# spcl/arrow-matrix

Measured on NVIDIA H100. Metric: iterated SpMM GFLOP/s (k=128), higher is better.
Workload: dtype f32

## Files before the change

arrow_matrix_b200/_lib.py:

```python
from __future__ import annotations

import ctypes
import os
from ctypes import (POINTER, byref, c_char_p, c_double, c_float, c_int, c_int32, c_int64, c_size_t, c_void_p)
from typing import Optional, Sequence, Tuple

import numpy as np

_HERE = os.path.dirname(os.path.abspath(__file__))
LIB_PATH = os.path.join(_HERE, "libarrow_b200.so")

ACCUMULATE = 1
F32, F64 = 0, 1
I32 = 2
B1 = 3
BITS = "bits"
_DTYPE_CODE = {np.dtype(np.float32): F32, np.dtype(np.float64): F64}
_TILE_CODE = {**_DTYPE_CODE, np.dtype(np.int32): I32}
_CODE_TILE = {**{c: dt for dt, c in _TILE_CODE.items()}, B1: BITS}
VARIANT_AUTO, VARIANT_DIRECT, VARIANT_SHFL, VARIANT_TMA, VARIANT_TILES = -1, 0, 1, 2, 3
SR_PLUS_TIMES, SR_MIN_PLUS, SR_MAX_PLUS, SR_OR_AND = 0, 1, 2, 3
SEMIRINGS = {"plus_times": SR_PLUS_TIMES, "min_plus": SR_MIN_PLUS, "max_plus": SR_MAX_PLUS, "or_and": SR_OR_AND}
IPC_HANDLE_BYTES = 80

# ... 8 lines not shown
    "arrow_event_record", "arrow_event_wait",
    "arrow_spmm", "arrow_spmm_add", "arrow_gather_rows", "arrow_gather_rows_multi",
    "arrow_ipc_export", "arrow_ipc_import", "arrow_peer_barrier",
    "arrow_timer_start", "arrow_timer_stop", "arrow_timer_elapsed_ms", "arrow_launch_count", "arrow_l2_flush",
    "arrow_ptrtable_upload", "arrow_ptrtable_free", "arrow_spmm_ex", "arrow_push_rows", "arrow_reduce_rows",
    "arrow_graph_begin", "arrow_graph_end", "arrow_graph_launch", "arrow_graph_free",
    "arrow_host_alloc_numa", "arrow_bind_thread_to_device_numa", "arrow_preload_kernels",
    "arrow_csr_upload_f64", "arrow_dense_alloc_dtype", "arrow_dense_dtype",
    "arrow_spmm_sr", "arrow_gather_rows_sr", "arrow_dense_count_diff",
    "arrow_spmm_sr_witness", "arrow_tile_rows", "arrow_tile_rows_rule", "arrow_bits_mark_new",
    "arrow_adj_build", "arrow_adj_free", "arrow_adj_info", "arrow_adj_d2h", "arrow_bits_mark_frontier",
    "arrow_bits_push_frontier", "arrow_adj_build_weighted", "arrow_adj_values_d2h", "arrow_sr_mark_frontier",
    "arrow_sr_push_frontier", "arrow_adj_build_in", "arrow_bits_parents", "arrow_bits_path_counts",
    "arrow_adj_keep_record", "arrow_bits_dependencies", "arrow_bits_fill_f64", "arrow_dense_row_sum",
    "arrow_adj_build_loopfree", "arrow_wpaths_counts", "arrow_wpaths_dependencies",
]
ABI_VERSION = 12


class ArrowError(RuntimeError):
    def __init__(self, code: int, message: str):
        super().__init__(f"libarrow_b200 error {code}: {message}")
        self.code = code


_lib = None


def load_library(build_if_missing: bool = True) -> ctypes.CDLL:
    global _lib
    if _lib is not None:
        return _lib
# ... 12 lines not shown
    I, I64 = c_int, c_int64
    pI, pI64 = POINTER(c_int), POINTER(c_int64)
    sig = {
        "arrow_b200_abi_version": (c_int, []),
        "arrow_ctx_create": (c_int, [I, P, POINTER(P)]),
        "arrow_ctx_destroy": (None, [P]),
        "arrow_last_error": (c_char_p, [P]),
        "arrow_sync": (c_int, [P]),
        "arrow_device_info": (c_int, [P, pI, pI64, pI64]),
        "arrow_set_tuning": (c_int, [P, I, I]),
        "arrow_set_option": (c_int, [P, I, I]),
        "arrow_csr_upload": (c_int, [P, I64, I64, I64, P, I, P, I, P, pI]),
        "arrow_csr_free": (c_int, [P, I]),
        "arrow_csr_info": (c_int, [P, I, pI64, pI64, pI64, pI64, pI64]),
        "arrow_csr_remap_columns": (c_int, [P, I, I, I64, pI]),
        "arrow_map_upload": (c_int, [P, P, I64, I64, pI]),
        "arrow_map_free": (c_int, [P, I]),
        "arrow_map_compose": (c_int, [P, I, I, pI]),
        "arrow_map_invert": (c_int, [P, I, I64, pI]),
        "arrow_map_d2h": (c_int, [P, I, P, I64]),
        "arrow_dense_alloc": (c_int, [P, I64, I, pI]),
        "arrow_dense_free": (c_int, [P, I]),
        "arrow_dense_fill": (c_int, [P, I, c_float]),
        "arrow_dense_h2d": (c_int, [P, I, I64, I64, P]),
        "arrow_dense_d2h": (c_int, [P, I, I64, I64, P]),
        "arrow_dense_copy": (c_int, [P, I, I64, I, I64, I64]),
        "arrow_dense_ptr": (c_int, [P, I, POINTER(P), pI64, pI]),
        "arrow_dense_wrap": (c_int, [P, P, I64, I, pI]),
        "arrow_dense_h2d_lane": (c_int, [P, I, I, I64, I64, P]),
        "arrow_dense_d2h_lane": (c_int, [P, I, I, I64, I64, P]),
        "arrow_lane_wait": (c_int, [P, I, I]),
        "arrow_lane_sync": (c_int, [P, I]),
        "arrow_set_lane": (c_int, [P, I]),
        "arrow_event_record": (c_int, [P, I, I]),
        "arrow_event_wait": (c_int, [P, I, I]),
        "arrow_host_alloc": (c_int, [c_size_t, POINTER(P)]),
        "arrow_host_free": (c_int, [P]),
        "arrow_spmm": (c_int, [P, I, I, I, I, I, I]),
        "arrow_spmm_add": (c_int, [P, I, I, I, I, I, I]),
        "arrow_gather_rows": (c_int, [P, I, I, I, I]),
        "arrow_gather_rows_multi": (c_int, [P, I, pI, pI64, I, I, I]),
        "arrow_ipc_export": (c_int, [P, I, P]),
        "arrow_ipc_import": (c_int, [P, P, I64, I, pI]),
        "arrow_peer_barrier": (c_int, [P, pI, I, I]),
        "arrow_timer_start": (c_int, [P, I]),
        "arrow_timer_stop": (c_int, [P, I]),
        "arrow_timer_elapsed_ms": (c_int, [P, I, POINTER(c_float)]),
        "arrow_launch_count": (c_int, [P, pI64]),
        "arrow_l2_flush": (c_int, [P]),
        "arrow_ptrtable_upload": (c_int, [P, pI, I, P, P, I64, pI]),
        "arrow_ptrtable_free": (c_int, [P, I]),
        "arrow_spmm_ex": (c_int, [P, I, I, I, I64, I, I, I, I, I]),
        "arrow_push_rows": (c_int, [P, pI, pI64, I, I, I]),
        "arrow_reduce_rows": (c_int, [P, I, I, pI, I, I64]),
# ... 226 lines not shown
    def ipc_import(self, handle: bytes, rows: int, k: int) -> "Dense":
        assert len(handle) == IPC_HANDLE_BYTES
        buf = ctypes.create_string_buffer(handle, IPC_HANDLE_BYTES)
        h = c_int()
        self._check(self.lib.arrow_ipc_import(self._h, buf, int(rows), int(k), byref(h)))
        return Dense(self, h.value, int(rows), int(k), owned=False)

    def spmm(self, A: "Csr", X: "Dense", C: "Dense", rowmap: Optional["RowMap"] = None,
             accumulate: bool = False, variant: int = VARIANT_AUTO):
        self._check(self.lib.arrow_spmm(self._h, A.h, X.h, C.h, rowmap.h if rowmap is not None else -1,
                                        ACCUMULATE if accumulate else 0, int(variant)))

    def spmm_add(self, A: "Csr", X: "Dense", C: "Dense", add: "Dense", add_map: "RowMap", variant: int = VARIANT_AUTO):
        self._check(self.lib.arrow_spmm_add(self._h, A.h, X.h, C.h, add.h, add_map.h, int(variant)))

    def spmm_sr(self, A: "Csr", X: "Dense", C: "Dense", add: Optional["Dense"] = None,
                add_map: Optional["RowMap"] = None, semiring: int = SR_PLUS_TIMES):
        self._check(self.lib.arrow_spmm_sr(self._h, A.h, X.h, C.h, add.h if add is not None else -1,
                                           add_map.h if add_map is not None else -1, int(semiring)))

    def spmm_sr_witness(self, A: "Csr", X: "Dense", labels: "Dense", values: Optional["Dense"] = None,
                        add_values: Optional["Dense"] = None, add_labels: Optional["Dense"] = None,
                        add_map: Optional["RowMap"] = None, dist: Optional["Dense"] = None,
                        row_labels: Optional["RowMap"] = None, semiring: int = SR_MIN_PLUS):
        h = lambda o: o.h if o is not None else -1
        self._check(self.lib.arrow_spmm_sr_witness(self._h, A.h, X.h, h(row_labels), h(values), labels.h, h(add_values),
                                                   h(add_labels), h(add_map), h(dist), int(semiring)))

    def spmm_ex(self, A: "Csr", X: "Dense", C: Optional["Dense"] = None, X2: Optional["Dense"] = None, x_split: int = 0,
                out_table: Optional["PtrTable"] = None, add: Optional["Dense"] = None, add_map: Optional["RowMap"] = None,
# ... 216 lines not shown
        self.n_rows, self.n_cols, self.nnz = n_rows, n_cols, nnz
        self.dtype = np.dtype(dtype)

    def info(self):
        v = [c_int64() for _ in range(5)]
        self.ctx._check(self.ctx.lib.arrow_csr_info(self.ctx._h, self.h, *[byref(x) for x in v]))
        return dict(zip(("n_rows", "n_cols", "nnz", "max_row_nnz", "n_long_rows"), (x.value for x in v)))

    def remap_columns(self, m: "RowMap", new_n_cols: int) -> "Csr":
        h = c_int()
        self.ctx._check(self.ctx.lib.arrow_csr_remap_columns(self.ctx._h, self.h, m.h, int(new_n_cols), byref(h)))
        out = Csr(self.ctx, h.value, self.n_rows, int(new_n_cols), self.nnz, self.dtype)
        out._parent = self
        return out

    def free(self):
        self._free("arrow_csr_free")


class RowMap(_Handle):
    def __init__(self, ctx, h, n, limit):
        super().__init__(ctx, h)
        self.n, self.limit = n, limit

    def compose(self, outer: "RowMap") -> "RowMap":
        h = c_int()
        self.ctx._check(self.ctx.lib.arrow_map_compose(self.ctx._h, self.h, outer.h, byref(h)))
        return RowMap(self.ctx, h.value, self.n, outer.limit)

    def invert(self, n_out: int) -> "RowMap":
# ... 95 lines not shown
```

arrow_matrix_b200/csrc/arrow_b200.cu:

```cuda
#include "../../include/arrow_b200.h"

#include <cuda_runtime.h>
#include <ctype.h>
#include <dlfcn.h>
#include <sched.h>
#include <sys/mman.h>
#include <sys/syscall.h>
#include <unistd.h>
#include <stdint.h>
#include <stdarg.h>
#include <stdio.h>
#include <string.h>

#include <cub/device/device_radix_sort.cuh>

#include <algorithm>
#include <map>
#include <mutex>
#include <type_traits>
#include <string>
#include <vector>

namespace {

struct DenseBuf {
    float *p = nullptr;
    int64_t rows = 0;
    int k = 0;
    int dtype = ARROW_F32;
// ... 1609 lines not shown
    bool bad = false;
    for (long long i = (long long)blockIdx.x * blockDim.x + threadIdx.x; i < n; i += stride) {
        const int c = idx[i];
        const int m = (c < 0 || c >= map_n) ? -1 : map[c];
        out[i] = m;
        bad = bad || m < 0;
    }
    if (bad && any_invalid != nullptr) atomicExch(any_invalid, 1);
}

__global__ void k_map_invert(const int *__restrict__ map, long long n, int *__restrict__ out, long long n_out) {
    const long long stride = (long long)gridDim.x * blockDim.x;
    for (long long i = (long long)blockIdx.x * blockDim.x + threadIdx.x; i < n; i += stride) {
        const int q = map[i];
        if (q >= 0 && q < n_out) out[q] = (int)i;
    }
}

struct PeerFlags {
    unsigned int *p[MAX_SRC];
};
__global__ void k_peer_barrier(PeerFlags flags, int rank, int world, unsigned int *epoch_ctr, int *status, long long timeout_clocks) {
    __shared__ unsigned int s_epoch;
    __threadfence_system();
    if (threadIdx.x == 0) {
        s_epoch = *epoch_ctr + 1u;
        *epoch_ctr = s_epoch;
    }
    __syncthreads();
    const unsigned int epoch = s_epoch;
// ... 2486 lines not shown
        if (e == cudaSuccess) e = cudaMemcpyAsync(&h_invalid, flag.p, sizeof(int), cudaMemcpyDeviceToHost, ctx->stream);
        if (e == cudaSuccess) e = cudaStreamSynchronize(ctx->stream);
    }
    if (e != cudaSuccess) {
        cudaFree(d.indices);
        return fail(ctx, ARROW_ERR_CUDA, "column remap failed: %s", cudaGetErrorString(e));
    }
    d.may_skip = c->may_skip || h_invalid != 0;
    const int h = new_slot(ctx->csrs);
    ctx->csrs[h] = d;
    ctx->csrs[csr].children++;
    *csr_out = h;
    return ARROW_OK;
}

int arrow_map_upload(arrow_ctx *ctx, const int64_t *map, int64_t n, int64_t limit, int *map_out) {
    CHECK_CTX(ctx);
    if (!map_out || (n > 0 && !map)) return fail(ctx, ARROW_ERR_ARG, "null pointer argument");
    if (n < 0 || limit < 0 || limit > 2147483647LL || n > 2147483647LL)
        return fail(ctx, ARROW_ERR_RANGE, "map size/limit exceed the int32 device layout");
    IdxMap m;
    m.n = n;
    m.limit = limit;
    CUDA_TRY(ctx, cudaMalloc(&m.p, (size_t)std::max<int64_t>(n, 1) * sizeof(int)));
    cudaError_t e = cudaSuccess;
    if (n > 0) {
        DevTmp wide;
        e = cudaMalloc(&wide.p, (size_t)n * 8);
        if (e == cudaSuccess) e = cudaMemcpyAsync(wide.p, map, (size_t)n * 8, cudaMemcpyHostToDevice, ctx->stream);
        if (e == cudaSuccess) {
// ... 242 lines not shown
    if (len) {
        const bool ok = cudaHostUnregister(ptr) == cudaSuccess;
        munmap(ptr, len);
        return ok ? ARROW_OK : ARROW_ERR_CUDA;
    }
    return cudaFreeHost(ptr) == cudaSuccess ? ARROW_OK : ARROW_ERR_CUDA;
}

struct SpmmCall {
    int csr = -1, x_buf = -1, c_buf = -1;
    int rowmap = -1, flags = 0, variant = ARROW_VARIANT_AUTO;
    int add_buf = -1, add_map = -1;
    int x2_buf = -1;
    int64_t x_split = 0;
    int out_table = -1;
};
static int spmm_impl(arrow_ctx *ctx, const SpmmCall &q);

#define CHECK_POISON(ctx)                                                                                     \
    do {                                                                                                      \
        if ((ctx)->poisoned) return fail((ctx), ARROW_ERR_CUDA, "context is poisoned by a peer-barrier time-out"); \
    } while (0)

int arrow_spmm(arrow_ctx *ctx, int csr, int x_buf, int c_buf, int rowmap, int flags, int variant) {
    SpmmCall q;
    q.csr = csr; q.x_buf = x_buf; q.c_buf = c_buf; q.rowmap = rowmap; q.flags = flags; q.variant = variant;
    return spmm_impl(ctx, q);
}

int arrow_spmm_add(arrow_ctx *ctx, int csr, int x_buf, int c_buf, int add_buf, int add_map, int variant) {
    SpmmCall q;
    q.csr = csr; q.x_buf = x_buf; q.c_buf = c_buf; q.variant = variant; q.add_buf = add_buf; q.add_map = add_map;
    return spmm_impl(ctx, q);
}

int arrow_spmm_ex(arrow_ctx *ctx, int csr, int x_buf, int x2_buf, int64_t x_split, int c_buf, int out_table,
                  int add_buf, int add_map, int variant) {
    SpmmCall q;
    q.csr = csr; q.x_buf = x_buf; q.x2_buf = x2_buf; q.x_split = x_split; q.c_buf = c_buf; q.out_table = out_table;
    q.add_buf = add_buf; q.add_map = add_map; q.variant = variant;
    return spmm_impl(ctx, q);
}

static int spmm_impl(arrow_ctx *ctx, const SpmmCall &q) {
    CHECK_CTX(ctx);
    CHECK_POISON(ctx);
    Csr *A = get_csr(ctx, q.csr);
// ... 75 lines not shown
        a.add_map = am->p;
    }
    if (A->dtype == ARROW_F64) {
        if (X2 || OT) return fail(ctx, ARROW_ERR_UNSUPPORTED, "float64 has no two-part X operand or pointer-table epilogue (one GPU only)");
        if (q.variant != ARROW_VARIANT_AUTO && q.variant != ARROW_VARIANT_TILES)
            return fail(ctx, ARROW_ERR_UNSUPPORTED, "float64 has no kernel variant override (variant %d)", q.variant);
        return spmm_f64(ctx, A, a, rm != nullptr, acc);
    }
    int variant = q.variant;
    if (variant == ARROW_VARIANT_AUTO) variant = pick_variant(k);
    const int vpl_req = (variant >> 4) & 0xF;
    const int rpg_req = (variant >> 8) & 0x3;
    variant &= 0xF;
    if ((a.add_map != nullptr || X2 || OT) && variant != 3) variant = 3;
    if (variant < 0 || variant > 3) return fail(ctx, ARROW_ERR_ARG, "unknown variant %d", variant);
    const bool fused_launch = rm != nullptr || acc || OT != nullptr || X2 != nullptr || a.add_map != nullptr;

    const bool vec_ok = (k % 4 == 0) && k <= 256;
    if (!vec_ok) {
        launch_generic<PlusTimes<float>>(ctx, a, rm != nullptr, acc);
    } else if (variant == 3) {
        if (A->n_tiles[TILE_LIST_SMALL] > 0) {
            TileArgs t;
            t.a = a;
            t.skip = (A->may_skip || ctx->force_skip_path) ? 1 : 0;
            t.ticket = ctx->tile_ticket + 2 * lane;
            t.l2_hints = (rm != nullptr || acc) ? ctx->l2_hints_fused : ctx->l2_hints_plain;
            t.prefetch = fused_launch ? ctx->prefetch_fused : ctx->prefetch_plain;
            TileLaunch L;
            L.out_mode = OT ? OUT_ROWPTR : (rm ? OUT_ROWMAP : OUT_IDENTITY);
            L.acc = acc;
            L.dualx = X2 != nullptr;
            L.vpl_req = vpl_req;
            L.rpg_req = rpg_req;
            int rc = launch_tiles(ctx, t, A, L);
            if (rc != ARROW_OK) return rc;
        }
    } else if (variant == ARROW_VARIANT_TMA && k >= 32 && k <= 128) {
        if (a.k4 <= 32) launch_tma<1>(ctx, a, rm != nullptr, acc);
        else launch_tma<2>(ctx, a, rm != nullptr, acc);
    } else {
        if (variant == ARROW_VARIANT_TMA) variant = ARROW_VARIANT_SHFL;
// ... 1747 lines not shown
```

arrow_matrix_b200/decomp.py:

```python
from __future__ import annotations

from typing import List, Optional, Sequence, Tuple, Union

import numpy as np
from scipy import sparse

Triplet = Tuple[Optional[np.ndarray], np.ndarray, np.ndarray]
Level = Union[sparse.csr_matrix, Triplet]


def level_triplet(level: Level) -> Triplet:
    if isinstance(level, tuple):
        return level
    m = sparse.csr_matrix(level)
    return (m.data, m.indices, m.indptr)


def number_of_blocks(level: Level, width: int) -> int:
    indptr = np.asarray(level_triplet(level)[2])
    nnz_total = int(indptr[-1] - indptr[0])
    if nnz_total == 0:
        raise ValueError("level has no non-zero row")
    last = int(np.searchsorted(indptr, indptr[-1], side="left")) - 1
    return -(-(last + 1) // width)
# ... 96 lines not shown
    assert ip.size == rows + 1
    out_ptr = ip + np.arange(rows + 1, dtype=np.int64)
    nnz = int(out_ptr[-1])
    diag = out_ptr[:-1]
    rest = np.ones(nnz, dtype=bool)
    rest[diag] = False
    idx = np.empty(nnz, dtype=np.result_type(np.asarray(indices).dtype, np.int32))
    idx[diag] = np.arange(rows)
    idx[rest] = indices
    dat = np.empty(nnz, dtype=dtype)
    dat[diag] = value
    dat[rest] = 1 if data is None else data
    return out_ptr, idx, dat


def block_partition(n_blocks: int, parts: int) -> np.ndarray:
    g = np.arange(parts + 1, dtype=np.int64)
    return (g * n_blocks + parts - 1) // parts


def locality_partition(to_prev: np.ndarray, n_blocks: int, width: int, prev_bounds_rows: np.ndarray, parts: int,
                       min_local: float = 0.5, max_skew: float = 4.0) -> Optional[np.ndarray]:
    rows = n_blocks * width
    if n_blocks < 1 or parts < 2:
        return None
    tp = np.asarray(to_prev[:rows])
    valid = tp < int(prev_bounds_rows[-1])
    owner = np.searchsorted(prev_bounds_rows, np.where(valid, tp, 0), side="right") - 1
    blk = np.arange(rows, dtype=np.int64) // width
    votes = np.zeros((n_blocks, parts), dtype=np.int64)
# ... 19 lines not shown
```

arrow_matrix_b200/engine.py:

```python
from __future__ import annotations

from typing import List, Optional, Sequence, Tuple

import numpy as np

from . import _lib
from . import decomp


_PLUS_ZERO = {_lib.SR_PLUS_TIMES: 0.0, _lib.SR_MIN_PLUS: float("inf"), _lib.SR_MAX_PLUS: float("-inf"), _lib.SR_OR_AND: 0.0}
_TIMES_ONE = {_lib.SR_PLUS_TIMES: 1.0, _lib.SR_MIN_PLUS: 0.0, _lib.SR_MAX_PLUS: 0.0, _lib.SR_OR_AND: 1.0}


BFS_PUSH_ALPHA = 8


def bfs_direction(frontier_edges: int, total_nnz: int, alpha: float = BFS_PUSH_ALPHA) -> str:
    return "push" if frontier_edges * alpha < total_nnz else "pull"


SR_PUSH_ALPHA = 9


def semiring_code(semiring: str, dtype, fused_style: str = "gather") -> int:
    if semiring not in _lib.SEMIRINGS:
        raise ValueError(f"unknown semiring {semiring!r}: expected one of {', '.join(_lib.SEMIRINGS)}")
    code = _lib.SEMIRINGS[semiring]
    if code != _lib.SR_PLUS_TIMES:
        if np.dtype(dtype) != np.float32:
            raise ValueError(f"the {semiring} semiring computes in float32, the decomposition is {np.dtype(dtype)}")
        if fused_style != "gather":
            raise ValueError(f"the {semiring} semiring runs the gather style of the fused step, not {fused_style!r}")
    return code


_SCAN_CHUNK = 1 << 24
# ... 2 lines not shown
def _nonpositive_edge(ip, idx, dat, cmap) -> bool:
    ip, idx, dat = np.asarray(ip), np.asarray(idx), np.asarray(dat)
    for e0 in range(0, dat.size, _SCAN_CHUNK):
        e = np.flatnonzero(~(dat[e0:e0 + _SCAN_CHUNK] > 0)) + e0
        if e.size == 0:
            continue
        r, c = np.searchsorted(ip, e, side="right") - 1, idx[e].astype(np.int64)
        ok = (r != c) & (c >= 0)
        if np.any(ok & (cmap[r] >= 0) & (cmap[np.where(ok, c, 0)] >= 0)):
            return True
    return False


class _LevelState:
    __slots__ = ("rows", "n_blocks", "csr", "csr_fused", "to_prev", "to_next_dev", "to_prev_dev", "cmap_dev",
                 "bufs", "xi", "ci", "nnz", "dropped", "cbuf")

    def __init__(self):
        self.csr = self.csr_fused = None
        self.to_prev = None
        self.to_prev_dev = self.to_next_dev = self.cmap_dev = None
        self.bufs = [None, None]
        self.xi = self.ci = 0
        self.cbuf = None


class ArrowEngine:

    def __init__(self, decomposition: Sequence[Tuple[decomp.Level, np.ndarray]], width: int, k: int,
                 block_diagonal: bool = True, device: int = 0, mode: str = "auto", stream: Optional[int] = None,
                 variant: int = _lib.VARIANT_AUTO, n_blocks: Optional[Sequence[int]] = None,
                 ctx: Optional[_lib.Context] = None, fused_style: str = "gather", dtype=np.float32,
                 semiring: str = "plus_times", add_identity: bool = False):
        if mode not in ("auto", "fused", "exchange"):
            raise ValueError(f"mode must be auto|fused|exchange, got {mode!r}")
        self.dtype = _lib.element_type(dtype)
        self.sr = semiring_code(semiring, self.dtype, fused_style)
        self.semiring = semiring
        self.add_identity = bool(add_identity)
# ... 18 lines not shown
        self.last_bfs_directions: List[str] = []
        self._adj: Optional[_lib.Adjacency] = None
        self._in_adj: Optional[_lib.Adjacency] = None
        self._bfs_parents: Optional[_lib.Dense] = None
        self._bfs_sigma: Optional[_lib.Dense] = None
        self._bfs_delta: Optional[Tuple[_lib.Dense, ...]] = None
        self._push_limit: Optional[int] = None
        self.last_fixed_point_directions: List[str] = []
        self._sr_adj: Optional[_lib.Adjacency] = None
        self._neg_zero_weight = False
        self._nonpos_weight = False
        self._wp_adjs: Optional[Tuple[_lib.Adjacency, ...]] = None
        self._wp_tiles: Optional[Tuple[_lib.Dense, ...]] = None
        self._wp_delta: Optional[Tuple[_lib.Dense, ...]] = None
        self.last_path_rounds = 0
        fused_ok = True
        cmap_prev = None
        for j, (B, _) in enumerate(decomposition):
            st = _LevelState()
            st.n_blocks = self.n_blocks[j]
            st.rows = st.n_blocks * width
            ip, idx, dat, dropped = decomp.arrow_rows(B, width, st.n_blocks, block_diagonal, 0, st.rows, dtype=self.dtype)
            st.dropped = dropped
            entries = (ip, idx, dat)
            if j == 0 and self.add_identity:
                ip, idx, dat = decomp.with_diagonal(ip, idx, dat, st.rows, _TIMES_ONE[self.sr], self.dtype)
            st.nnz = int(ip[-1])
            if self.sr in (_lib.SR_MIN_PLUS, _lib.SR_MAX_PLUS) and np.any((dat == 0) & np.signbit(dat)):
                self._neg_zero_weight = True
            st.csr = self.ctx.csr_upload(st.rows, st.rows, ip, idx, dat, dtype=self.dtype)
# ... 33 lines not shown
    def _alloc(self, rows: int) -> _lib.Dense:
        b = self.ctx.dense_alloc(rows, self.k, _lib.BITS if self.bits else self.dtype)
        if _PLUS_ZERO[self.sr] != 0.0:
            b.fill(_PLUS_ZERO[self.sr])
        return b

    def _alloc_buffers(self):
        for j, st in enumerate(self.levels):
            if j == 0 or self.mode == "exchange":
                st.bufs = [self._alloc(st.rows), self._alloc(st.rows)]
                st.xi, st.ci = 0, 0
            if j > 0 and self.mode == "fused":
                st.csr_fused = st.csr.remap_columns(st.cmap_dev, self.levels[0].rows)
                if self.fused_style == "gather":
                    st.cbuf = self._alloc(st.rows)

    def set_mode(self, mode: str):
        if mode == self.mode:
            return
        if mode == "fused" and not self.fused_ok:
            raise ValueError("fused mode is not valid for this decomposition")
        if hasattr(self, "_slots"):
            self.stream_drain()
            for b in self._slots[1]:
                b.free()
            self.levels[0].bufs = list(self._slots[0])
            del self._slots
        for st in self.levels:
            for b in st.bufs:
                if b is not None:
                    b.free()
            st.bufs = [None, None]
            if st.csr_fused is not None:
                st.csr_fused.free()
                st.csr_fused = None
            if st.cbuf is not None:
                st.cbuf.free()
                st.cbuf = None
        self.mode = mode
        self._alloc_buffers()

    @property
# ... 77 lines not shown

    def sync(self):
        if hasattr(self, "_slots"):
            self.stream_drain()
        self.ctx.sync()

    def _product(self, A: _lib.Csr, X: _lib.Dense, C: _lib.Dense, add: Optional[_lib.Dense] = None,
                 add_map: Optional[_lib.RowMap] = None):
        if self.sr != _lib.SR_PLUS_TIMES:
            self.ctx.spmm_sr(A, X, C, add, add_map, self.sr)
        elif add is None:
            self.ctx.spmm(A, X, C, variant=self.variant)
        else:
            self.ctx.spmm_add(A, X, C, add, add_map, variant=self.variant)

    def propagate_features(self):
        if self.mode == "fused":
            return
        for j in range(1, self.L):
            st, prev = self.levels[j], self.levels[j - 1]
            self.ctx.gather_rows(st.bufs[st.ci], prev.bufs[prev.xi], st.to_prev_dev)
            st.xi = st.ci

    def spmm(self):
        if self.mode == "fused":
            st0 = self.levels[0]
            x = st0.bufs[st0.xi]
            out = 1 - st0.xi
            if self.fused_style == "gather":
                for j in range(self.L - 1, 0, -1):
                    st = self.levels[j]
                    if j == self.L - 1:
                        self._product(st.csr_fused, x, st.cbuf)
                    else:
                        nxt = self.levels[j + 1]
                        self._product(st.csr_fused, x, st.cbuf, nxt.cbuf, nxt.to_next_dev)
                if self.L > 1:
                    nxt = self.levels[1]
                    self._product(st0.csr, x, st0.bufs[out], nxt.cbuf, nxt.to_next_dev)
                else:
                    self._product(st0.csr, x, st0.bufs[out])
            else:
                self.ctx.spmm(st0.csr, x, st0.bufs[out], variant=self.variant)
                for st in self.levels[1:]:
                    self.ctx.spmm(st.csr_fused, x, st0.bufs[out], rowmap=st.cmap_dev, accumulate=True,
                                  variant=self.variant)
            st0.ci = out
            return
        for st in self.levels:
            out = 1 - st.xi
            self._product(st.csr, st.bufs[st.xi], st.bufs[out])
            st.ci = out

    def aggregate(self):
        if self.mode == "fused":
            st0 = self.levels[0]
# ... 343 lines not shown
            return 4, 4.0 * _lib.b1_words(self.k)
        e = self.dtype.itemsize
        return 4 + e, float(self.k * e)

    def algorithmic_bytes_per_step(self) -> float:
        nz, row = self._entry_and_row_bytes()
        total = 0.0
        for j, st in enumerate(self.levels):
            total += st.nnz * nz + (st.rows + 1) * 4 + 2.0 * st.rows * row
            if j > 0:
                m = int(np.count_nonzero(st.to_prev < self.levels[j - 1].rows))
                total += 5.0 * m * row
        return total

    def _launch_level_as_in_step(self, j: int, src, dst):
        st = self.levels[j]
        if self.mode == "fused" and self.fused_style == "gather" and j + 1 < self.L:
            nxt = self.levels[j + 1]
            self._product(st.csr, src, dst, nxt.cbuf, nxt.to_next_dev)
        else:
            self._product(st.csr, src, dst)

    def time_level_spmm(self, j: int, iters: int, warmup: int = 3) -> float:
        st = self.levels[j]
        if j > 0 and self.mode == "fused":
            raise ValueError("levels > 0 are timed through step() in fused mode")
        src = st.bufs[st.xi]
        scratch = self._alloc(st.rows)
        for _ in range(warmup):
            self._launch_level_as_in_step(j, src, scratch)
        self.ctx.timer_start(5)
        for _ in range(iters):
            self._launch_level_as_in_step(j, src, scratch)
        self.ctx.timer_stop(5)
        ms = self.ctx.timer_ms(5) / iters
        scratch.free()
# ... 9 lines not shown
        return b

    def close(self):
        for b in (self._wit_labels or []) + list(self._wit_values.values()) + list(self._bfs_tiles or ()):
            b.free()
        for a in (self._adj, self._sr_adj, self._in_adj, self._bfs_parents):
            if a is not None:
                a.free()
        self._wit_labels, self._wit_values, self._bfs_tiles, self._adj, self._sr_adj = None, {}, None, None, None
        for b in (self._bfs_sigma,) + (self._bfs_delta or ()) + (self._wp_adjs or ()) + (self._wp_tiles or ()) + \
                (self._wp_delta or ()):
            if b is not None:
                b.free()
        self._in_adj = self._bfs_parents = self._bfs_sigma = self._bfs_delta = None
        self._wp_adjs = self._wp_tiles = self._wp_delta = None
        self.ctx.close()
```

include/arrow_b200.h:

```cpp
#ifndef ARROW_B200_H
#define ARROW_B200_H

#include <stdint.h>
#include <stddef.h>

#ifdef __cplusplus
extern "C" {
#endif

typedef struct arrow_ctx arrow_ctx;

#define ARROW_ABI_VERSION 12

#define ARROW_OK              0
#define ARROW_ERR_CUDA       -1
#define ARROW_ERR_ARG        -2
#define ARROW_ERR_HANDLE     -3
#define ARROW_ERR_RANGE      -4
#define ARROW_ERR_NOMEM      -5
#define ARROW_ERR_UNSUPPORTED -6

#define ARROW_F32             0
#define ARROW_F64             1
#define ARROW_I32             2
#define ARROW_B1              3

#define ARROW_ACCUMULATE      1
// ... 30 lines not shown
int  arrow_tile_rows(arrow_ctx *ctx, int k, int dtype, int *rows);
int  arrow_tile_rows_rule(int k, int elem_bytes, int64_t l2_bytes, int resident_ctas, int big_ok);

int  arrow_csr_upload(arrow_ctx *ctx, int64_t n_rows, int64_t n_cols, int64_t nnz,
                      const void *indptr, int indptr_bytes,
                      const void *indices, int indices_bytes,
                      const float *data, int *csr_out);
int  arrow_csr_upload_f64(arrow_ctx *ctx, int64_t n_rows, int64_t n_cols, int64_t nnz,
                          const void *indptr, int indptr_bytes,
                          const void *indices, int indices_bytes,
                          const double *data, int *csr_out);
int  arrow_csr_free(arrow_ctx *ctx, int csr);
int  arrow_csr_info(arrow_ctx *ctx, int csr, int64_t *n_rows, int64_t *n_cols, int64_t *nnz,
                    int64_t *max_row_nnz, int64_t *n_long_rows);
int  arrow_csr_remap_columns(arrow_ctx *ctx, int csr, int map, int64_t new_n_cols, int *csr_out);

int  arrow_map_upload(arrow_ctx *ctx, const int64_t *map, int64_t n, int64_t limit, int *map_out);
int  arrow_map_free(arrow_ctx *ctx, int map);
int  arrow_map_compose(arrow_ctx *ctx, int inner, int outer, int *map_out);
int  arrow_map_invert(arrow_ctx *ctx, int map, int64_t n_out, int *map_out);
int  arrow_map_d2h(arrow_ctx *ctx, int map, int32_t *host, int64_t n);

int  arrow_dense_alloc(arrow_ctx *ctx, int64_t rows, int k, int *buf_out);
int  arrow_dense_alloc_dtype(arrow_ctx *ctx, int64_t rows, int k, int dtype, int *buf_out);
int  arrow_dense_dtype(arrow_ctx *ctx, int buf, int *dtype);
int  arrow_dense_free(arrow_ctx *ctx, int buf);
int  arrow_dense_fill(arrow_ctx *ctx, int buf, float value);
int  arrow_dense_h2d(arrow_ctx *ctx, int buf, int64_t row0, int64_t rows, const void *host);
int  arrow_dense_d2h(arrow_ctx *ctx, int buf, int64_t row0, int64_t rows, void *host);
int  arrow_dense_copy(arrow_ctx *ctx, int dst, int64_t dst_row0, int src, int64_t src_row0, int64_t rows);
// ... 8 lines not shown
int  arrow_dense_d2h_lane(arrow_ctx *ctx, int lane, int buf, int64_t row0, int64_t rows, void *host);
int  arrow_lane_wait(arrow_ctx *ctx, int waiting_lane, int signalling_lane);
int  arrow_lane_sync(arrow_ctx *ctx, int lane);
int  arrow_set_lane(arrow_ctx *ctx, int lane);
#define ARROW_MAX_EVENTS 16
int  arrow_event_record(arrow_ctx *ctx, int event, int lane);
int  arrow_event_wait(arrow_ctx *ctx, int event, int lane);
int  arrow_host_alloc(size_t bytes, void **ptr);
int  arrow_host_free(void *ptr);
int  arrow_host_alloc_numa(size_t bytes, int device, void **ptr);
int  arrow_bind_thread_to_device_numa(int device, int *node_out, int *n_cpus_out);

int  arrow_spmm(arrow_ctx *ctx, int csr, int x_buf, int c_buf, int rowmap, int flags, int variant);

int  arrow_spmm_add(arrow_ctx *ctx, int csr, int x_buf, int c_buf, int add_buf, int add_map, int variant);

int  arrow_gather_rows(arrow_ctx *ctx, int dst_buf, int src_buf, int map, int flags);

#define ARROW_SR_PLUS_TIMES 0
#define ARROW_SR_MIN_PLUS   1
#define ARROW_SR_MAX_PLUS   2
#define ARROW_SR_OR_AND     3
int  arrow_spmm_sr(arrow_ctx *ctx, int csr, int x_buf, int c_buf, int add_buf, int add_map, int semiring);
int  arrow_gather_rows_sr(arrow_ctx *ctx, int dst_buf, int src_buf, int map, int semiring);
int  arrow_dense_count_diff(arrow_ctx *ctx, int a, int b, int64_t *rows_changed);
int  arrow_bits_mark_new(arrow_ctx *ctx, int new_buf, int old_buf, int dist_buf, int level, int64_t *n_new);

int  arrow_adj_build(arrow_ctx *ctx, int n_parts, const int *csrs, const int *maps, int64_t n_vertices, int *adj_out);
int  arrow_adj_free(arrow_ctx *ctx, int adj);
int  arrow_adj_info(arrow_ctx *ctx, int adj, int64_t *n_vertices, int64_t *n_edges);
// ... 66 lines not shown
```

Before: 3854.

## Reorder fused-level CSR rows by first column within block rows for locality

Adds a GPU-built row schedule that permutes the short rows of each fused level's CSR within block-row groups, sorted by first column index. Output goes back to the original rows through an output row map. The aim is better reuse of gathered X rows in L2 and cache across neighbouring warps. The fused gather path in the engine uses these scheduled CSRs by default when k is at least 64 and the dtype is f32. The cost is an indirect output write and one extra map compose for the add path, plus extra memory for a second CSR copy per level.

```diff
diff --git a/arrow_matrix_b200/_lib.py b/arrow_matrix_b200/_lib.py
--- a/arrow_matrix_b200/_lib.py
+++ b/arrow_matrix_b200/_lib.py
@@ -46,8 +46,9 @@
     "arrow_sr_push_frontier", "arrow_adj_build_in", "arrow_bits_parents", "arrow_bits_path_counts",
     "arrow_adj_keep_record", "arrow_bits_dependencies", "arrow_bits_fill_f64", "arrow_dense_row_sum",
     "arrow_adj_build_loopfree", "arrow_wpaths_counts", "arrow_wpaths_dependencies",
+    "arrow_csr_row_schedule", "arrow_spmm_rows",
 ]
-ABI_VERSION = 12
+ABI_VERSION = 13
 
 
 class ArrowError(RuntimeError):
@@ -90,6 +91,7 @@
         "arrow_csr_free": (c_int, [P, I]),
         "arrow_csr_info": (c_int, [P, I, pI64, pI64, pI64, pI64, pI64]),
         "arrow_csr_remap_columns": (c_int, [P, I, I, I64, pI]),
+        "arrow_csr_row_schedule": (c_int, [P, I, I64, pI, pI]),
         "arrow_map_upload": (c_int, [P, P, I64, I64, pI]),
         "arrow_map_free": (c_int, [P, I]),
         "arrow_map_compose": (c_int, [P, I, I, pI]),
@@ -114,6 +116,7 @@
         "arrow_host_free": (c_int, [P]),
         "arrow_spmm": (c_int, [P, I, I, I, I, I, I]),
         "arrow_spmm_add": (c_int, [P, I, I, I, I, I, I]),
+        "arrow_spmm_rows": (c_int, [P, I, I, I, I, I, I, I]),
         "arrow_gather_rows": (c_int, [P, I, I, I, I]),
         "arrow_gather_rows_multi": (c_int, [P, I, pI, pI64, I, I, I]),
         "arrow_ipc_export": (c_int, [P, I, P]),
@@ -370,6 +373,11 @@
     def spmm_add(self, A: "Csr", X: "Dense", C: "Dense", add: "Dense", add_map: "RowMap", variant: int = VARIANT_AUTO):
         self._check(self.lib.arrow_spmm_add(self._h, A.h, X.h, C.h, add.h, add_map.h, int(variant)))
 
+    def spmm_rows(self, A: "Csr", X: "Dense", C: "Dense", out_rows: "RowMap", add: Optional["Dense"] = None,
+                  add_map: Optional["RowMap"] = None, variant: int = VARIANT_AUTO):
+        self._check(self.lib.arrow_spmm_rows(self._h, A.h, X.h, C.h, out_rows.h, add.h if add is not None else -1,
+                                             add_map.h if add_map is not None else -1, int(variant)))
+
     def spmm_sr(self, A: "Csr", X: "Dense", C: "Dense", add: Optional["Dense"] = None,
                 add_map: Optional["RowMap"] = None, semiring: int = SR_PLUS_TIMES):
         self._check(self.lib.arrow_spmm_sr(self._h, A.h, X.h, C.h, add.h if add is not None else -1,
@@ -616,6 +624,12 @@
         out._parent = self
         return out
 
+    def row_schedule(self, width: int) -> Tuple["Csr", "RowMap"]:
+        h, m = c_int(), c_int()
+        self.ctx._check(self.ctx.lib.arrow_csr_row_schedule(self.ctx._h, self.h, int(width), byref(h), byref(m)))
+        return (Csr(self.ctx, h.value, self.n_rows, self.n_cols, self.nnz, self.dtype),
+                RowMap(self.ctx, m.value, self.n_rows, self.n_rows))
+
     def free(self):
         self._free("arrow_csr_free")
 
diff --git a/arrow_matrix_b200/csrc/arrow_b200.cu b/arrow_matrix_b200/csrc/arrow_b200.cu
--- a/arrow_matrix_b200/csrc/arrow_b200.cu
+++ b/arrow_matrix_b200/csrc/arrow_b200.cu
@@ -13,6 +13,9 @@
 #include <string.h>
 
 #include <cub/device/device_radix_sort.cuh>
+#include <cub/device/device_scan.cuh>
+#include <cub/device/device_select.cuh>
+#include <thrust/iterator/counting_iterator.h>
 
 #include <algorithm>
 #include <map>
@@ -1652,6 +1655,45 @@
     for (long long i = (long long)blockIdx.x * blockDim.x + threadIdx.x; i < n; i += stride) {
         const int q = map[i];
         if (q >= 0 && q < n_out) out[q] = (int)i;
+    }
+}
+
+__global__ void k_sched_keys(const int *__restrict__ indptr, const int *__restrict__ indices, long long n_rows,
+                             long long width, int thr, unsigned long long *__restrict__ keys,
+                             unsigned char *__restrict__ movable, int *__restrict__ perm) {
+    const long long stride = (long long)gridDim.x * blockDim.x;
+    for (long long r = (long long)blockIdx.x * blockDim.x + threadIdx.x; r < n_rows; r += stride) {
+        const int s = indptr[r], e = indptr[r + 1];
+        const bool mv = r >= width && e > s && e - s <= thr;
+        movable[r] = mv ? 1 : 0;
+        keys[r] = ((unsigned long long)(r / width) << 32) | (unsigned int)(mv ? indices[s] : 0);
+        perm[r] = (int)r;
+    }
+}
+
+__global__ void k_sched_scatter(const int *__restrict__ pos, const int *__restrict__ rows, long long m, int *__restrict__ perm) {
+    const long long stride = (long long)gridDim.x * blockDim.x;
+    for (long long i = (long long)blockIdx.x * blockDim.x + threadIdx.x; i < m; i += stride) perm[pos[i]] = rows[i];
+}
+
+__global__ void k_sched_lens(const int *__restrict__ indptr, const int *__restrict__ perm, long long n, int *__restrict__ lens) {
+    const long long stride = (long long)gridDim.x * blockDim.x;
+    for (long long p = (long long)blockIdx.x * blockDim.x + threadIdx.x; p < n; p += stride)
+        lens[p] = indptr[perm[p] + 1] - indptr[perm[p]];
+}
+
+__global__ void k_sched_copy(const int *__restrict__ indptr, const int *__restrict__ indices, const float *__restrict__ vals,
+                             const int *__restrict__ perm, const int *__restrict__ new_ptr, long long n,
+                             int *__restrict__ out_idx, float *__restrict__ out_vals) {
+    const int lane = threadIdx.x & 31;
+    const long long warps = (long long)gridDim.x * (blockDim.x >> 5);
+    for (long long p = (long long)blockIdx.x * (blockDim.x >> 5) + (threadIdx.x >> 5); p < n; p += warps) {
+        const int r = perm[p];
+        const int s = indptr[r], len = indptr[r + 1] - s, d = new_ptr[p];
+        for (int i = lane; i < len; i += 32) {
+            out_idx[d + i] = indices[s + i];
+            out_vals[d + i] = vals[s + i];
+        }
     }
 }
 
@@ -4168,6 +4210,115 @@
     return ARROW_OK;
 }
 
+static int row_schedule_fill(arrow_ctx *ctx, const Csr &c, int64_t width, Csr &d, int *perm) {
+    cudaStream_t s = ctx->stream;
+    const long long n = c.n_rows;
+    const int grid = ctx->sm_count * 8;
+    d.dtype = c.dtype;
+    d.n_rows = c.n_rows;
+    d.n_cols = c.n_cols;
+    d.nnz = c.nnz;
+    d.may_skip = c.may_skip;
+    d.owns_indptr = d.owns_indices = d.owns_vals = d.owns_long = true;
+    CUDA_TRY(ctx, cudaMalloc(&d.indptr, ((size_t)n + 1 + 8) * sizeof(int)));
+    CUDA_TRY(ctx, cudaMemsetAsync(d.indptr, 0, ((size_t)n + 1 + 8) * sizeof(int), s));
+    const size_t nz = (size_t)c.nnz + 8;
+    CUDA_TRY(ctx, cudaMalloc(&d.indices, nz * sizeof(int)));
+    CUDA_TRY(ctx, cudaMalloc(&d.vals, nz * sizeof(float)));
+    CUDA_TRY(ctx, cudaMemsetAsync(d.indices, 0, nz * sizeof(int), s));
+    CUDA_TRY(ctx, cudaMemsetAsync(d.vals, 0, nz * sizeof(float), s));
+    DevTmp keys, mkeys, flags, pos, rows_sorted, count, lens, temp;
+    CUDA_TRY(ctx, cudaMalloc(&keys.p, (size_t)n * 8 + 8));
+    CUDA_TRY(ctx, cudaMalloc(&mkeys.p, (size_t)n * 8 + 8));
+    CUDA_TRY(ctx, cudaMalloc(&flags.p, (size_t)n + 8));
+    CUDA_TRY(ctx, cudaMalloc(&pos.p, (size_t)n * 4 + 8));
+    CUDA_TRY(ctx, cudaMalloc(&rows_sorted.p, (size_t)n * 4 + 8));
+    CUDA_TRY(ctx, cudaMalloc(&count.p, sizeof(int)));
+    CUDA_TRY(ctx, cudaMalloc(&lens.p, ((size_t)n + 1) * 4));
+    unsigned long long *kp = reinterpret_cast<unsigned long long *>(keys.p);
+    unsigned long long *km = reinterpret_cast<unsigned long long *>(mkeys.p);
+    unsigned char *fp = reinterpret_cast<unsigned char *>(flags.p);
+    int *pp = reinterpret_cast<int *>(pos.p);
+    int *rs = reinterpret_cast<int *>(rows_sorted.p);
+    int *np = reinterpret_cast<int *>(count.p);
+    int *lp = reinterpret_cast<int *>(lens.p);
+    k_sched_keys<<<grid, 256, 0, s>>>(c.indptr, c.indices, n, width, c.long_threshold, kp, fp, perm);
+    ctx->launches++;
+    CUDA_TRY(ctx, cudaGetLastError());
+    int end_bit = 33;
+    while (end_bit < 64 && (1LL << (end_bit - 32)) <= (n - 1) / width) ++end_bit;
+    thrust::counting_iterator<int> ids(0);
+    size_t b0 = 0, b1 = 0, b2 = 0, b3 = 0;
+    CUDA_TRY(ctx, cub::DeviceSelect::Flagged(nullptr, b0, kp, fp, km, np, (int)n, s));
+    CUDA_TRY(ctx, cub::DeviceSelect::Flagged(nullptr, b1, ids, fp, pp, np, (int)n, s));
+    CUDA_TRY(ctx, cub::DeviceRadixSort::SortPairs(nullptr, b2, km, kp, pp, rs, (int)n, 0, end_bit, s));
+    CUDA_TRY(ctx, cub::DeviceScan::ExclusiveSum(nullptr, b3, lp, d.indptr, (int)n + 1, s));
+    const size_t temp_bytes = std::max(std::max(b0, b1), std::max(b2, b3));
+    CUDA_TRY(ctx, cudaMalloc(&temp.p, std::max<size_t>(temp_bytes, 1)));
+    int m = 0;
+    size_t tb = temp_bytes;
+    CUDA_TRY(ctx, cub::DeviceSelect::Flagged(temp.p, tb, kp, fp, km, np, (int)n, s));
+    tb = temp_bytes;
+    CUDA_TRY(ctx, cub::DeviceSelect::Flagged(temp.p, tb, ids, fp, pp, np, (int)n, s));
+    CUDA_TRY(ctx, cudaMemcpyAsync(&m, np, sizeof(int), cudaMemcpyDeviceToHost, s));
+    CUDA_TRY(ctx, cudaStreamSynchronize(s));
+    if (m > 0) {
+        tb = temp_bytes;
+        CUDA_TRY(ctx, cub::DeviceRadixSort::SortPairs(temp.p, tb, km, kp, pp, rs, m, 0, end_bit, s));
+        k_sched_scatter<<<grid, 256, 0, s>>>(pp, rs, m, perm);
+        ctx->launches++;
+    }
+    k_sched_lens<<<grid, 256, 0, s>>>(c.indptr, perm, n, lp);
+    ctx->launches++;
+    CUDA_TRY(ctx, cudaMemsetAsync(lp + n, 0, sizeof(int), s));
+    tb = temp_bytes;
+    CUDA_TRY(ctx, cub::DeviceScan::ExclusiveSum(temp.p, tb, lp, d.indptr, (int)n + 1, s));
+    k_sched_copy<<<grid, 256, 0, s>>>(c.indptr, c.indices, c.vals, perm, d.indptr, n, d.indices, d.vals);
+    ctx->launches++;
+    CUDA_TRY(ctx, cudaGetLastError());
+    std::vector<int> h_indptr((size_t)n + 1);
+    CUDA_TRY(ctx, cudaMemcpyAsync(h_indptr.data(), d.indptr, ((size_t)n + 1) * sizeof(int), cudaMemcpyDeviceToHost, s));
+    CUDA_TRY(ctx, cudaStreamSynchronize(s));
+    const int rc = build_long_rows(ctx, d, h_indptr);
+    if (rc != ARROW_OK) return rc;
+    CUDA_TRY(ctx, cudaStreamSynchronize(s));
+    return ARROW_OK;
+}
+
+int arrow_csr_row_schedule(arrow_ctx *ctx, int csr, int64_t width, int *csr_out, int *map_out) {
+    CHECK_CTX(ctx);
+    Csr *c = get_csr(ctx, csr);
+    if (!c) return fail(ctx, ARROW_ERR_HANDLE, "bad csr handle %d", csr);
+    if (!csr_out || !map_out) return fail(ctx, ARROW_ERR_ARG, "null pointer argument");
+    if (width < 1) return fail(ctx, ARROW_ERR_ARG, "block-row width must be >= 1, got %lld", (long long)width);
+    if (c->dtype != ARROW_F32) return fail(ctx, ARROW_ERR_UNSUPPORTED, "row schedules exist for float32 blocks only");
+    if (c->long_threshold != ctx->long_threshold)
+        return fail(ctx, ARROW_ERR_ARG, "the long-row threshold changed since csr %d was built (%d, now %d)", csr,
+                    c->long_threshold, ctx->long_threshold);
+    IdxMap m;
+    m.n = c->n_rows;
+    m.limit = c->n_rows;
+    CUDA_TRY(ctx, cudaMalloc(&m.p, (size_t)std::max<int64_t>(m.n, 1) * sizeof(int)));
+    Csr d;
+    const int rc = row_schedule_fill(ctx, *c, width, d, m.p);
+    if (rc != ARROW_OK) {
+        cudaStreamSynchronize(ctx->stream);
+        cudaGetLastError();
+        csr_release(d);
+        cudaFree(m.p);
+        return rc;
+    }
+    d.live = true;
+    const int h = new_slot(ctx->csrs);
+    ctx->csrs[h] = d;
+    m.live = true;
+    const int hm = new_slot(ctx->maps);
+    ctx->maps[hm] = m;
+    *csr_out = h;
+    *map_out = hm;
+    return ARROW_OK;
+}
+
 int arrow_map_upload(arrow_ctx *ctx, const int64_t *map, int64_t n, int64_t limit, int *map_out) {
     CHECK_CTX(ctx);
     if (!map_out || (n > 0 && !map)) return fail(ctx, ARROW_ERR_ARG, "null pointer argument");
@@ -4440,6 +4591,7 @@
     int x2_buf = -1;
     int64_t x_split = 0;
     int out_table = -1;
+    bool scheduled = false;
 };
 static int spmm_impl(arrow_ctx *ctx, const SpmmCall &q);
 
@@ -4457,6 +4609,14 @@
 int arrow_spmm_add(arrow_ctx *ctx, int csr, int x_buf, int c_buf, int add_buf, int add_map, int variant) {
     SpmmCall q;
     q.csr = csr; q.x_buf = x_buf; q.c_buf = c_buf; q.variant = variant; q.add_buf = add_buf; q.add_map = add_map;
+    return spmm_impl(ctx, q);
+}
+
+int arrow_spmm_rows(arrow_ctx *ctx, int csr, int x_buf, int c_buf, int out_rows, int add_buf, int add_map, int variant) {
+    if (out_rows < 0) return fail(ctx, ARROW_ERR_HANDLE, "bad out-row map handle %d", out_rows);
+    SpmmCall q;
+    q.csr = csr; q.x_buf = x_buf; q.c_buf = c_buf; q.rowmap = out_rows; q.scheduled = true; q.variant = variant;
+    q.add_buf = add_buf; q.add_map = add_map;
     return spmm_impl(ctx, q);
 }
 
@@ -4562,7 +4722,8 @@
     variant &= 0xF;
     if ((a.add_map != nullptr || X2 || OT) && variant != 3) variant = 3;
     if (variant < 0 || variant > 3) return fail(ctx, ARROW_ERR_ARG, "unknown variant %d", variant);
-    const bool fused_launch = rm != nullptr || acc || OT != nullptr || X2 != nullptr || a.add_map != nullptr;
+    const bool scatter = (rm != nullptr && !q.scheduled) || acc;
+    const bool fused_launch = scatter || OT != nullptr || X2 != nullptr || a.add_map != nullptr;
 
     const bool vec_ok = (k % 4 == 0) && k <= 256;
     if (!vec_ok) {
@@ -4573,7 +4734,7 @@
             t.a = a;
             t.skip = (A->may_skip || ctx->force_skip_path) ? 1 : 0;
             t.ticket = ctx->tile_ticket + 2 * lane;
-            t.l2_hints = (rm != nullptr || acc) ? ctx->l2_hints_fused : ctx->l2_hints_plain;
+            t.l2_hints = scatter ? ctx->l2_hints_fused : ctx->l2_hints_plain;
             t.prefetch = fused_launch ? ctx->prefetch_fused : ctx->prefetch_plain;
             TileLaunch L;
             L.out_mode = OT ? OUT_ROWPTR : (rm ? OUT_ROWMAP : OUT_IDENTITY);
diff --git a/arrow_matrix_b200/decomp.py b/arrow_matrix_b200/decomp.py
--- a/arrow_matrix_b200/decomp.py
+++ b/arrow_matrix_b200/decomp.py
@@ -134,6 +134,17 @@
     return out_ptr, idx, dat
 
 
+def row_schedule(indptr: np.ndarray, indices: np.ndarray, width: int, long_threshold: int) -> np.ndarray:
+    ip = np.asarray(indptr, dtype=np.int64)
+    n = ip.size - 1
+    lens = np.diff(ip)
+    mv = np.flatnonzero((np.arange(n) >= width) & (lens > 0) & (lens <= long_threshold))
+    col0 = np.asarray(indices)[ip[mv]].astype(np.int64) & 0xFFFFFFFF
+    perm = np.arange(n, dtype=np.int64)
+    perm[mv] = mv[np.lexsort((mv, col0, mv // width))]
+    return perm
+
+
 def block_partition(n_blocks: int, parts: int) -> np.ndarray:
     g = np.arange(parts + 1, dtype=np.int64)
     return (g * n_blocks + parts - 1) // parts
diff --git a/arrow_matrix_b200/engine.py b/arrow_matrix_b200/engine.py
--- a/arrow_matrix_b200/engine.py
+++ b/arrow_matrix_b200/engine.py
@@ -20,6 +20,9 @@
 
 
 SR_PUSH_ALPHA = 9
+
+
+ROW_SCHEDULE_MIN_K = 64
 
 
 def semiring_code(semiring: str, dtype, fused_style: str = "gather") -> int:
@@ -52,7 +55,7 @@
 
 class _LevelState:
     __slots__ = ("rows", "n_blocks", "csr", "csr_fused", "to_prev", "to_next_dev", "to_prev_dev", "cmap_dev",
-                 "bufs", "xi", "ci", "nnz", "dropped", "cbuf")
+                 "bufs", "xi", "ci", "nnz", "dropped", "cbuf", "sched")
 
     def __init__(self):
         self.csr = self.csr_fused = None
@@ -61,6 +64,7 @@
         self.bufs = [None, None]
         self.xi = self.ci = 0
         self.cbuf = None
+        self.sched = None
 
 
 class ArrowEngine:
@@ -109,6 +113,7 @@
         self._wp_tiles: Optional[Tuple[_lib.Dense, ...]] = None
         self._wp_delta: Optional[Tuple[_lib.Dense, ...]] = None
         self.last_path_rounds = 0
+        self._row_schedule = True
         fused_ok = True
         cmap_prev = None
         for j, (B, _) in enumerate(decomposition):
@@ -172,6 +177,24 @@
                 st.csr_fused = st.csr.remap_columns(st.cmap_dev, self.levels[0].rows)
                 if self.fused_style == "gather":
                     st.cbuf = self._alloc(st.rows)
+        if self.mode == "fused" and self.fused_style == "gather" and self.sr == _lib.SR_PLUS_TIMES and \
+                self.dtype == np.float32 and self.k >= ROW_SCHEDULE_MIN_K:
+            self._build_row_schedules()
+
+    def _build_row_schedules(self):
+        for j, st in enumerate(self.levels):
+            if j == 0:
+                continue
+            csr, rows = st.csr_fused.row_schedule(self.width)
+            add_map = rows.compose(self.levels[j + 1].to_next_dev) if j + 1 < self.L else None
+            st.sched = (csr, rows, add_map)
+
+    def _free_row_schedules(self):
+        for st in self.levels:
+            for h in st.sched or ():
+                if h is not None:
+                    h.free()
+            st.sched = None
 
     def set_mode(self, mode: str):
         if mode == self.mode:
@@ -184,6 +207,7 @@
                 b.free()
             self.levels[0].bufs = list(self._slots[0])
             del self._slots
+        self._free_row_schedules()
         for st in self.levels:
             for b in st.bufs:
                 if b is not None:
@@ -291,6 +315,17 @@
         else:
             self.ctx.spmm_add(A, X, C, add, add_map, variant=self.variant)
 
+    def _gather_launch(self, j: int, x: _lib.Dense, dst: _lib.Dense):
+        st = self.levels[j]
+        nxt = self.levels[j + 1] if j + 1 < self.L else None
+        if st.sched is not None and self._row_schedule:
+            csr, rows, add_map = st.sched
+            self.ctx.spmm_rows(csr, x, dst, rows, nxt.cbuf if nxt is not None else None, add_map, variant=self.variant)
+        elif nxt is None:
+            self._product(st.csr if j == 0 else st.csr_fused, x, dst)
+        else:
+            self._product(st.csr if j == 0 else st.csr_fused, x, dst, nxt.cbuf, nxt.to_next_dev)
+
     def propagate_features(self):
         if self.mode == "fused":
             return
@@ -306,17 +341,8 @@
             out = 1 - st0.xi
             if self.fused_style == "gather":
                 for j in range(self.L - 1, 0, -1):
-                    st = self.levels[j]
-                    if j == self.L - 1:
-                        self._product(st.csr_fused, x, st.cbuf)
-                    else:
-                        nxt = self.levels[j + 1]
-                        self._product(st.csr_fused, x, st.cbuf, nxt.cbuf, nxt.to_next_dev)
-                if self.L > 1:
-                    nxt = self.levels[1]
-                    self._product(st0.csr, x, st0.bufs[out], nxt.cbuf, nxt.to_next_dev)
-                else:
-                    self._product(st0.csr, x, st0.bufs[out])
+                    self._gather_launch(j, x, self.levels[j].cbuf)
+                self._gather_launch(0, x, st0.bufs[out])
             else:
                 self.ctx.spmm(st0.csr, x, st0.bufs[out], variant=self.variant)
                 for st in self.levels[1:]:
@@ -690,12 +716,10 @@
         return total
 
     def _launch_level_as_in_step(self, j: int, src, dst):
-        st = self.levels[j]
-        if self.mode == "fused" and self.fused_style == "gather" and j + 1 < self.L:
-            nxt = self.levels[j + 1]
-            self._product(st.csr, src, dst, nxt.cbuf, nxt.to_next_dev)
+        if self.mode == "fused" and self.fused_style == "gather":
+            self._gather_launch(j, src, dst)
         else:
-            self._product(st.csr, src, dst)
+            self._product(self.levels[j].csr, src, dst)
 
     def time_level_spmm(self, j: int, iters: int, warmup: int = 3) -> float:
         st = self.levels[j]
@@ -735,4 +759,5 @@
                 b.free()
         self._in_adj = self._bfs_parents = self._bfs_sigma = self._bfs_delta = None
         self._wp_adjs = self._wp_tiles = self._wp_delta = None
+        self._free_row_schedules()
         self.ctx.close()
diff --git a/include/arrow_b200.h b/include/arrow_b200.h
--- a/include/arrow_b200.h
+++ b/include/arrow_b200.h
@@ -10,7 +10,7 @@
 
 typedef struct arrow_ctx arrow_ctx;
 
-#define ARROW_ABI_VERSION 12
+#define ARROW_ABI_VERSION 13
 
 #define ARROW_OK              0
 #define ARROW_ERR_CUDA       -1
@@ -71,6 +71,7 @@
 int  arrow_csr_info(arrow_ctx *ctx, int csr, int64_t *n_rows, int64_t *n_cols, int64_t *nnz,
                     int64_t *max_row_nnz, int64_t *n_long_rows);
 int  arrow_csr_remap_columns(arrow_ctx *ctx, int csr, int map, int64_t new_n_cols, int *csr_out);
+int  arrow_csr_row_schedule(arrow_ctx *ctx, int csr, int64_t width, int *csr_out, int *map_out);
 
 int  arrow_map_upload(arrow_ctx *ctx, const int64_t *map, int64_t n, int64_t limit, int *map_out);
 int  arrow_map_free(arrow_ctx *ctx, int map);
@@ -109,6 +110,8 @@
 int  arrow_spmm(arrow_ctx *ctx, int csr, int x_buf, int c_buf, int rowmap, int flags, int variant);
 
 int  arrow_spmm_add(arrow_ctx *ctx, int csr, int x_buf, int c_buf, int add_buf, int add_map, int variant);
+
+int  arrow_spmm_rows(arrow_ctx *ctx, int csr, int x_buf, int c_buf, int out_rows, int add_buf, int add_map, int variant);
 
 int  arrow_gather_rows(arrow_ctx *ctx, int dst_buf, int src_buf, int map, int flags);
 
```

Result: faster. 3925 (median of 6 runs) (+1.9%).
